# BigCiLeng/bilateral-driving

Measured on AMD Instinct MI355X. Metric: train iters/sec (fwd+bwd) at 2M Gaussians, 6x1920x1080; HBM roofline %, higher is better.
Workload: dtype f32

## Files before the change

bilateral_driving_amd/csrc/tiles.hip:

```cpp
#include "bds_common.h"
#include "gs_math.h"

namespace bds {

constexpr int kScanBlock = 256;
constexpr int kScanItems = 8;
constexpr int kScanTile = kScanBlock * kScanItems;

__device__ __forceinline__ uint32_t wave_incl_scan(uint32_t v) {
  const int lane = threadIdx.x & (kWave - 1);
#pragma unroll
  for (int o = 1; o < kWave; o <<= 1) {
    uint32_t t = __shfl_up(v, o);
    if (lane >= o) v += t;
  }
  return v;
}

__device__ __forceinline__ uint32_t block_excl_scan(uint32_t v, uint32_t &total, uint32_t *lds_w ) {
  const int lane = threadIdx.x & (kWave - 1), wv = threadIdx.x / kWave;
  const int nw = blockDim.x / kWave;
  uint32_t inc = wave_incl_scan(v);
  if (lane == kWave - 1) lds_w[wv] = inc;
  __syncthreads();
// ... 378 lines not shown
          gt[u] += c;
          if (g < gb) below[u] += c;
        }
      }
      const uint32_t *hp = hist + ((int64_t)gb << kWideGroupShift) * kBins + tid * kPer;
      const int nrows = vb - (gb << kWideGroupShift);
      uint32_t p0[kPer], p1[kPer], p2[kPer], p3[kPer];
#pragma unroll
      for (int u = 0; u < kPer; u++) { p0[u] = 0; p1[u] = 0; p2[u] = 0; p3[u] = 0; }
      int r = 0;
      for (; r + 4 <= nrows; r += 4) {
        const uint32_t *q = hp + (int64_t)r * kBins;
#pragma unroll
        for (int u = 0; u < kPer; u++) { p0[u] += q[u]; p1[u] += q[kBins + u]; p2[u] += q[2 * kBins + u]; p3[u] += q[3 * kBins + u]; }
      }
      for (; r < nrows; r++) {
#pragma unroll
        for (int u = 0; u < kPer; u++) p0[u] += hp[(int64_t)r * kBins + u];
      }
#pragma unroll
      for (int u = 0; u < kPer; u++) below[u] += (p0[u] + p1[u]) + (p2[u] + p3[u]);
    }
    uint32_t gsum = 0;
#pragma unroll
    for (int u = 0; u < kPer; u++) gsum += gt[u];
    uint32_t all;
    uint32_t dbase = block_excl_scan(gsum, all, lw);
    uint32_t base = block_excl_scan(sum, all, lw);
#pragma unroll
    for (int u = 0; u < kPer; u++) {
      const int d = tid * kPer + u;
      dstart[d] = base;
      gbase[d] = dbase + below[u];
      dbase += gt[u];
      if (offsets_out && vb == 0 && d < n_offsets) offsets_out[d] = (int32_t)gbase[d];
      uint32_t b2 = base;
#pragma unroll
      for (int w = 0; w < kSortWaves; w++) {
        const uint32_t c = wrun[w][d];
        wrun[w][d] = b2;
        b2 += c;
      }
      base += tot[u];
    }
  }
  __syncthreads();
  const unsigned long long lt = lane == 0 ? 0ull : (~0ull >> (64 - lane));
#pragma unroll
  for (int r = 0; r < kSortRounds; r++) {
    const int64_t i = wbase + r * kWave + lane;
    const bool on = i < n;
    const uint32_t d = (k[r] >> shift) & mask;
    unsigned long long peers = __ballot(on);
    for (int b = 0; b < bits; b++) {
      const unsigned long long bal = __ballot((d >> b) & 1u);
      peers &= ((d >> b) & 1u) ? bal : ~bal;
    }
    const uint32_t rank = __popcll(peers & lt);
    uint32_t pos = 0;
    if (on) pos = wrun[wv][d];
    __builtin_amdgcn_s_waitcnt(0xc07f);
    __builtin_amdgcn_wave_barrier();
    if (on && rank == 0) wrun[wv][d] = pos + __popcll(peers);
    __builtin_amdgcn_wave_barrier();
    if (on) lk[pos + rank] = k[r];
  }
  __syncthreads();
  const int cnt = (int)((n - bbase) < (int64_t)kSortChunk ? (n - bbase) : (int64_t)kSortChunk);
  for (int i = tid; i < cnt; i += kSortBlock) {
    const uint32_t kk = lk[i];
    const uint32_t d = (kk >> shift) & mask;
    const uint32_t g = gbase[d] + ((uint32_t)i - dstart[d]);
    keys_out[g] = kk;
    if (unpack) vals_out[g] = unpack[kk & rank_mask];
  }
}
template <int kBins>
__global__ __launch_bounds__(kSortBlock) void radix_scatter_keys_wide_kernel(
    const uint32_t *__restrict__ keys_in, int64_t n_host, const uint64_t *__restrict__ n_dev, int shift, uint32_t mask, int bits,
    const uint32_t *__restrict__ hist, const uint32_t *__restrict__ ghist, uint32_t *__restrict__ keys_out,
    const uint32_t *__restrict__ unpack, uint32_t rank_mask, uint32_t *__restrict__ vals_out, int32_t *__restrict__ offsets_out,
    int n_offsets) {
  __shared__ ScatterWideSh<kBins> sh;
  radix_scatter_keys_wide_block<kBins>(sh, (int)blockIdx.x, keys_in, list_length(n_host, n_dev), shift, mask, bits, hist, ghist, keys_out,
                                       unpack, rank_mask, vals_out, offsets_out, n_offsets);
}

constexpr int kWideBits = 10;

static size_t radix_temp_elems(int64_t n, int max_bins = 256) {
  const int64_t nblocks = cdiv(n > 0 ? n : 1, kSortChunk);
  const size_t h = align_up((size_t)max_bins * nblocks, 4);
  const size_t group_rows = max_bins > 256 ? (size_t)max_bins * (size_t)cdiv(nblocks, 1 << kWideGroupShift) : 0;
  const size_t behind = scan_temp_elems((int64_t)max_bins * nblocks);
  return h + (behind > group_rows ? behind : group_rows);
}

static size_t radix_wide_group_elems(int64_t n, int bits) {
  return (size_t)(1 << bits) * (size_t)cdiv(cdiv(n > 0 ? n : 1, kSortChunk), 1 << kWideGroupShift);
}

static int radix_pass(const uint32_t *kin, const uint32_t *vin, uint32_t *kout, uint32_t *vout, int64_t n, int shift,
                      int bits, uint32_t *temp, hipStream_t st, const uint64_t *n_dev = nullptr) {
  if (n == 0) return BDS_OK;
  const int nblocks = (int)cdiv(n, kSortChunk);
  const uint32_t mask = (1u << bits) - 1u;
  const int64_t hn = (int64_t)(mask + 1) * nblocks;
  uint32_t *hist = temp;
  uint32_t *stemp = temp + align_up((size_t)256 * nblocks, 4);
  hipLaunchKernelGGL(radix_hist_kernel, dim3(nblocks), dim3(kSortBlock), 0, st, kin, n, n_dev, shift, mask, nblocks, hist);
  BDS_LAUNCH_CHECK();
  int rc = exclusive_scan_u32(hist, hist, hn, stemp, nullptr, st);
  if (rc != BDS_OK) return rc;
  hipLaunchKernelGGL(radix_scatter_lds_kernel, dim3(nblocks), dim3(kSortBlock), 0, st, kin, vin, n, n_dev, shift, mask, bits,
                     nblocks, hist, kout, vout);
  BDS_LAUNCH_CHECK();
  return BDS_OK;
}


static int radix_pass_keys(const uint32_t *kin, uint32_t *kout, int64_t n, int shift, int bits, uint32_t *temp, hipStream_t st,
                           const uint32_t *unpack, uint32_t rank_mask, uint32_t *vout, int32_t *offsets_out = nullptr,
                           int n_offsets = 0, const uint64_t *n_dev = nullptr) {
  if (n == 0) return BDS_OK;
  const int nblocks = (int)cdiv(n, kSortChunk);
  const uint32_t mask = (1u << bits) - 1u;
  const int64_t hn = (int64_t)(mask + 1) * nblocks;
  uint32_t *hist = temp;
  uint32_t *stemp = temp + align_up((size_t)(bits > 8 ? (1 << kWideBits) : 256) * nblocks, 4);
  if (bits > 8) {
    uint32_t *ghist = stemp;
    if (bits == 9) {
      hipLaunchKernelGGL((radix_hist_wide_kernel<512>), dim3(nblocks), dim3(kSortBlock), 0, st, kin, n, n_dev, shift, mask, hist, ghist);
      hipLaunchKernelGGL((radix_scatter_keys_wide_kernel<512>), dim3(nblocks), dim3(kSortBlock), 0, st, kin, n, n_dev, shift, mask, bits,
                         hist, ghist, kout, unpack, rank_mask, vout, offsets_out, n_offsets);
    } else {
      hipLaunchKernelGGL((radix_hist_wide_kernel<1024>), dim3(nblocks), dim3(kSortBlock), 0, st, kin, n, n_dev, shift, mask, hist, ghist);
      hipLaunchKernelGGL((radix_scatter_keys_wide_kernel<1024>), dim3(nblocks), dim3(kSortBlock), 0, st, kin, n, n_dev, shift, mask, bits,
                         hist, ghist, kout, unpack, rank_mask, vout, offsets_out, n_offsets);
    }
    BDS_LAUNCH_CHECK();
    return BDS_OK;
  }
  hipLaunchKernelGGL(radix_hist_kernel, dim3(nblocks), dim3(kSortBlock), 0, st, kin, n, n_dev, shift, mask, nblocks, hist);
  BDS_LAUNCH_CHECK();
  int rc = exclusive_scan_u32(hist, hist, hn, stemp, nullptr, st);
  if (rc != BDS_OK) return rc;
  hipLaunchKernelGGL(radix_scatter_keys_kernel, dim3(nblocks), dim3(kSortBlock), 0, st, kin, n, n_dev, shift, mask, bits, nblocks,
                     hist, kout, unpack, rank_mask, vout);
  BDS_LAUNCH_CHECK();
  return BDS_OK;
}

constexpr int kGroupShift = 6;
constexpr int kShortRounds = 4;
constexpr int kShortChunk = kSortBlock * kShortRounds;
constexpr int kChunkShift = 10;
static_assert(kShortChunk == (1 << kChunkShift), "chunk shift");
constexpr int64_t kShortSortMax = (int64_t)kShortChunk * 8192;

struct ShortHistSh { uint32_t h[256]; };
__device__ __forceinline__ void short_hist_block(ShortHistSh &sh, int vb, const uint32_t *keys, int64_t n, int shift,
                                                 uint32_t *hist , uint32_t *ghist ) {
  const int64_t base = (int64_t)vb * kShortChunk;
  if (base >= n) return;
  sh.h[threadIdx.x] = 0;
  __syncthreads();
#pragma unroll 4
  for (int r = 0; r < kShortRounds; r++) {
    const int64_t i = base + r * kSortBlock + threadIdx.x;
    if (i < n) atomicAdd(&sh.h[(keys[i] >> shift) & 255u], 1u);
  }
  __syncthreads();
  const uint32_t c = sh.h[threadIdx.x];
  hist[(int64_t)vb * 256 + threadIdx.x] = c;
  if (c) atomicAdd(&ghist[(int64_t)(vb >> kGroupShift) * 256 + threadIdx.x], c);
}
__device__ __forceinline__ int64_t bounded_count(const uint64_t *n_dev, int64_t n_cap) {
  const int64_t n = (int64_t)*n_dev;
  return (n_cap >= 0 && n > n_cap) ? 0 : n;
}
__global__ __launch_bounds__(kSortBlock) void short_hist_kernel(const uint32_t *__restrict__ keys,
                                                               const uint64_t *__restrict__ n_dev, int64_t n_cap, int shift,
                                                               uint32_t *__restrict__ hist ,
                                                               uint32_t *__restrict__ ghist ) {
  __shared__ ShortHistSh sh;
  short_hist_block(sh, (int)blockIdx.x, keys, bounded_count(n_dev, n_cap), shift, hist, ghist);
}

struct ShortScatterSh {
  uint32_t wrun[kSortWaves][256];
  uint32_t lw[kSortBlock / kWave + 1];
};
__device__ __forceinline__ void short_scatter_block(ShortScatterSh &sh, int vb, const uint32_t *keys_in, const uint32_t *vals_in, int64_t n,
                                                    int shift, const uint32_t *hist, const uint32_t *ghist, uint32_t *keys_out,
                                                    uint32_t *vals_out) {
  if ((int64_t)vb * kShortChunk >= n) return;
  auto &wrun = sh.wrun;
  uint32_t *lw = sh.lw;
  const int tid = threadIdx.x, lane = tid & (kWave - 1), wv = tid / kWave;
#pragma unroll
  for (int w = 0; w < kSortWaves; w++) wrun[w][tid] = 0;
  const int nb = (int)((n + kShortChunk - 1) >> kChunkShift), ng = (nb + (1 << kGroupShift) - 1) >> kGroupShift;
  const int gb = vb >> kGroupShift;
  uint32_t below = 0, total = 0;
  {
    int g = 0;
    for (; g + 4 <= ng; g += 4) {
      const uint32_t *q = ghist + (int64_t)g * 256 + tid;
      const uint32_t c0 = q[0], c1 = q[256], c2 = q[512], c3 = q[768];
      total += (c0 + c1) + (c2 + c3);
      below += (g < gb ? c0 : 0u) + (g + 1 < gb ? c1 : 0u) + (g + 2 < gb ? c2 : 0u) + (g + 3 < gb ? c3 : 0u);
    }
    for (; g < ng; g++) {
      const uint32_t c = ghist[(int64_t)g * 256 + tid];
      total += c;
      if (g < gb) below += c;
    }
  }
  {
    const uint32_t *hp = hist + ((int64_t)gb << kGroupShift) * 256 + tid;
    const int nrows = vb - (gb << kGroupShift);
    uint32_t p0 = 0, p1 = 0, p2 = 0, p3 = 0, p4 = 0, p5 = 0, p6 = 0, p7 = 0;
    int r = 0;
    for (; r + 8 <= nrows; r += 8) {
      const uint32_t *q = hp + (int64_t)r * 256;
      const uint32_t a0 = q[0], a1 = q[256], a2 = q[512], a3 = q[768], a4 = q[1024], a5 = q[1280], a6 = q[1536], a7 = q[1792];
      p0 += a0; p1 += a1; p2 += a2; p3 += a3; p4 += a4; p5 += a5; p6 += a6; p7 += a7;
    }
    for (; r < nrows; r++) p0 += hp[(int64_t)r * 256];
    below += ((p0 + p1) + (p2 + p3)) + ((p4 + p5) + (p6 + p7));
  }
  uint32_t all;
  const uint32_t digit_base = block_excl_scan(total, all, lw);
  constexpr int kPerWave = kShortChunk / kSortWaves;
  const int64_t wbase = (int64_t)vb * kShortChunk + (int64_t)wv * kPerWave;
  uint32_t k[kShortRounds], v[kShortRounds];
#pragma unroll
  for (int r = 0; r < kShortRounds; r++) {
    const int64_t i = wbase + r * kWave + lane;
    k[r] = 0xFFFFFFFFu; v[r] = 0;
    if (i < n) {
      k[r] = keys_in[i]; v[r] = vals_in[i];
      atomicAdd(&wrun[wv][(k[r] >> shift) & 255u], 1u);
    }
  }
  __syncthreads();
  {
    uint32_t base = digit_base + below;
#pragma unroll
    for (int w = 0; w < kSortWaves; w++) {
      const uint32_t c = wrun[w][tid];
      wrun[w][tid] = base;
      base += c;
    }
  }
  __syncthreads();
  const unsigned long long lt = lane == 0 ? 0ull : (~0ull >> (64 - lane));
#pragma unroll
  for (int r = 0; r < kShortRounds; r++) {
    const int64_t i = wbase + r * kWave + lane;
    const bool on = i < n;
    const uint32_t d = (k[r] >> shift) & 255u;
    unsigned long long peers = __ballot(on);
#pragma unroll
    for (int b = 0; b < 8; b++) {
      const unsigned long long bal = __ballot((d >> b) & 1u);
      peers &= ((d >> b) & 1u) ? bal : ~bal;
    }
    const uint32_t rank = __popcll(peers & lt);
    uint32_t pos = 0;
    if (on) pos = wrun[wv][d];
    __builtin_amdgcn_s_waitcnt(0xc07f);
    __builtin_amdgcn_wave_barrier();
    if (on && rank == 0) wrun[wv][d] = pos + __popcll(peers);
    __builtin_amdgcn_wave_barrier();
    if (on) {
      keys_out[pos + rank] = k[r];
      vals_out[pos + rank] = v[r];
    }
  }
}
__global__ __launch_bounds__(kSortBlock) void short_scatter_kernel(
    const uint32_t *__restrict__ keys_in, const uint32_t *__restrict__ vals_in, const uint64_t *__restrict__ n_dev, int64_t n_cap,
    int shift, const uint32_t *__restrict__ hist, const uint32_t *__restrict__ ghist, uint32_t *__restrict__ keys_out,
    uint32_t *__restrict__ vals_out) {
  __shared__ ShortScatterSh sh;
  short_scatter_block(sh, (int)blockIdx.x, keys_in, vals_in, bounded_count(n_dev, n_cap), shift, hist, ghist, keys_out, vals_out);
}

static size_t short_sort_elems(int64_t n_bound) {
  const int64_t nb = cdiv(n_bound > 0 ? n_bound : 1, kShortChunk), ng = cdiv(nb, 1 << kGroupShift);
  return (size_t)(nb + 4 * ng) * 256;
}

constexpr int kIsectBlock = 256;

__global__ __launch_bounds__(kIsectBlock) void isect_flag_kernel(int64_t CN, const int32_t *__restrict__ radii,
                                                                uint32_t *__restrict__ flags) {
  const int64_t o = (int64_t)blockIdx.x * kIsectBlock + threadIdx.x;
  if (o < CN) flags[o] = radii[o] > 0 ? 1u : 0u;
}

__global__ __launch_bounds__(kIsectBlock) void isect_compact_kernel(int64_t CN, const int32_t *__restrict__ radii,
                                                                   const uint32_t *__restrict__ pos,
                                                                   const float *__restrict__ depths,
                                                                   uint32_t *__restrict__ keys, uint32_t *__restrict__ vals,
                                                                   uint32_t *__restrict__ asc, int compact, int sd) {
  const int64_t o = (int64_t)blockIdx.x * kIsectBlock + threadIdx.x;
  if (o >= CN || radii[o] <= 0) return;
  const uint32_t j = pos[o];
  keys[j] = __float_as_uint(depths[o * sd]);
  vals[j] = compact ? j : (uint32_t)o;
  asc[j] = (uint32_t)o;
}

__global__ __launch_bounds__(kScanBlock) void visible_reduce_kernel(int64_t CN, const int32_t *__restrict__ radii,
                                                                   uint32_t *__restrict__ tile_sums,
                                                                   uint32_t *__restrict__ zero_me, int64_t zero_elems,
                                                                   uint64_t *__restrict__ m_total, int32_t *__restrict__ zero_cn) {
  __shared__ uint32_t lw[kScanBlock / kWave + 1];
  if (blockIdx.x == 0 && threadIdx.x == 0) *m_total = 0;
  for (int64_t i = (int64_t)blockIdx.x * kScanBlock + threadIdx.x; i < zero_elems; i += (int64_t)gridDim.x * kScanBlock)
    zero_me[i] = 0u;
  const int64_t base = (int64_t)blockIdx.x * kScanTile + (int64_t)threadIdx.x * kScanItems;
  uint32_t s = 0;
#pragma unroll
  for (int i = 0; i < kScanItems; i++) {
    if (base + i < CN) {
      s += radii[base + i] > 0 ? 1u : 0u;
      if (zero_cn) zero_cn[base + i] = 0;
    }
  }
  uint32_t tot;
  block_excl_scan(s, tot, lw);
  if (threadIdx.x == 0) tile_sums[blockIdx.x] = tot;
}

constexpr int kCompactSpan = kScanTile / kShortChunk + 1;
struct VisCompactSh {
  uint32_t lw[kScanBlock / kWave + 1];
  uint32_t h[kCompactSpan][256];
};
__device__ __forceinline__ void visible_compact_block(VisCompactSh &sh, int vb, int nvb, int64_t CN, const int32_t *radii, const float *depths,
                                                      const uint32_t *tile_sums, uint32_t *keys, uint32_t *vals, uint32_t *hist,
                                                      uint32_t *ghist, uint64_t *n_vis_out, uint32_t *asc, int compact, int sums_per_tile,
                                                      int sd) {
  constexpr int kSpan = kCompactSpan;
  uint32_t *lw = sh.lw;
  auto &h = sh.h;
#pragma unroll
  for (int t = 0; t < kSpan; t++) h[t][threadIdx.x] = 0;
  uint32_t part = 0;
  for (int b = threadIdx.x; b < vb * sums_per_tile; b += kScanBlock) part += tile_sums[b];
  uint32_t my_offset;
  block_excl_scan(part, my_offset, lw);
  const int64_t base = (int64_t)vb * kScanTile + (int64_t)threadIdx.x * kScanItems;
  bool vis[kScanItems];
  uint32_t s = 0;
#pragma unroll
  for (int i = 0; i < kScanItems; i++) {
    vis[i] = base + i < CN && radii[base + i] > 0;
    s += vis[i] ? 1u : 0u;
  }
  uint32_t tot;
  uint32_t j = block_excl_scan(s, tot, lw) + my_offset;
  const uint32_t chunk0 = my_offset >> kChunkShift;
#pragma unroll
  for (int i = 0; i < kScanItems; i++) {
    if (vis[i]) {
      const uint32_t key = __float_as_uint(depths[(base + i) * sd]);
      keys[j] = key;
      vals[j] = compact ? j : (uint32_t)(base + i);
      asc[j] = (uint32_t)(base + i);
      atomicAdd(&h[(j >> kChunkShift) - chunk0][key & 255u], 1u);
      j++;
    }
  }
  __syncthreads();
#pragma unroll
  for (int t = 0; t < kSpan; t++) {
    const uint32_t c = h[t][threadIdx.x];
    if (c) {
      atomicAdd(&hist[(int64_t)(chunk0 + t) * 256 + threadIdx.x], c);
      atomicAdd(&ghist[(int64_t)((chunk0 + t) >> kGroupShift) * 256 + threadIdx.x], c);
    }
  }
  if (vb == nvb - 1 && threadIdx.x == 0) *n_vis_out = (uint64_t)my_offset + tot;
}
__global__ __launch_bounds__(kScanBlock) void visible_compact_kernel(int64_t CN, const int32_t *__restrict__ radii,
                                                                    const float *__restrict__ depths,
                                                                    const uint32_t *__restrict__ tile_sums,
                                                                    uint32_t *__restrict__ keys, uint32_t *__restrict__ vals,
                                                                    uint32_t *__restrict__ hist, uint32_t *__restrict__ ghist,
                                                                    uint64_t *__restrict__ n_vis_out, uint32_t *__restrict__ asc,
                                                                    int compact, int sums_per_tile, int sd) {
  __shared__ VisCompactSh sh;
  visible_compact_block(sh, (int)blockIdx.x, (int)gridDim.x, CN, radii, depths, tile_sums, keys, vals, hist, ghist, n_vis_out, asc, compact,
                        sums_per_tile, sd);
}

struct RowStage {
  float mx[kIsectBlock], my[kIsectBlock], a[kIsectBlock], b[kIsectBlock], c[kIsectBlock], qmax[kIsectBlock];
  int x0[kIsectBlock], x1[kIsectBlock], y0[kIsectBlock];
  uint32_t id[kIsectBlock];
  uint32_t cam_base[kIsectBlock];
  uint32_t rowoff[kIsectBlock + 1];
  uint32_t lw[kIsectBlock / kWave + 1];
};

constexpr int kRecWords = 12;

__device__ __forceinline__ uint32_t stage_rows(RowStage &S, int64_t j0, int64_t n_vis, int64_t N, const uint32_t *__restrict__ sorted_idx,
                                               const uint32_t *__restrict__ asc ,
                                               const float *__restrict__ means2d, const int32_t *__restrict__ radii,
                                               const float *__restrict__ conics, const float *__restrict__ opacities,
                                               int tile_size, int tile_w, int tile_h, float4 *__restrict__ rec_out,
                                               const float4 *__restrict__ rec_in, const ProjLayout pl) {
  const int t = threadIdx.x;
  const int64_t j = j0 + t;
  uint32_t nrows = 0;
  if (j < n_vis) {
    if (rec_in != nullptr) {
      const float4 r0 = rec_in[j * 3], r1 = rec_in[j * 3 + 1], r2 = rec_in[j * 3 + 2];
      nrows = __float_as_uint(r2.y);
      S.mx[t] = r0.x; S.my[t] = r0.y; S.a[t] = r0.z; S.b[t] = r0.w;
      S.c[t] = r1.x; S.qmax[t] = r1.y; S.x0[t] = __float_as_int(r1.z); S.x1[t] = __float_as_int(r1.w);
      S.y0[t] = __float_as_int(r2.x); S.id[t] = __float_as_uint(r2.z); S.cam_base[t] = __float_as_uint(r2.w);
    } else {
      const uint32_t val = sorted_idx[j];
      const uint32_t o = asc ? asc[val] : val;
      const int r = proj_radius(pl, means2d, radii, (int64_t)o);
      float mx = means2d[(int64_t)o * pl.s2], my = means2d[(int64_t)o * pl.s2 + 1];
      float a = 0.f, b = 0.f, c = 0.f, q_max = 0.f, op = 0.f;
      if (conics != nullptr) {
        a = conics[(int64_t)o * pl.sc]; b = conics[(int64_t)o * pl.sc + 1]; c = conics[(int64_t)o * pl.sc + 2];
        op = opacities[(int64_t)o * pl.so];
      }
      int x0 = 0, y0 = 0, x1 = 0, y1 = 0;
      if (r > 0) {
        bool ok;
        if (conics == nullptr) {
          tile_rect(mx, my, r, tile_size, tile_w, tile_h, x0, y0, x1, y1);
          ok = x1 > x0 && y1 > y0;
        } else {
          ok = tile_rect_tight(mx, my, r, a, b, c, op, tile_size, tile_w, tile_h, x0, y0, x1, y1, q_max);
        }
        if (ok) nrows = (uint32_t)(y1 - y0);
      } else {
        mx = my = a = b = c = 0.f;
      }
      const uint32_t cam_base = (int64_t)o < N ? 0u : (uint32_t)((uint32_t)o / (uint32_t)N) * (uint32_t)(tile_w * tile_h);
      S.mx[t] = mx; S.my[t] = my; S.a[t] = a; S.b[t] = b; S.c[t] = c; S.qmax[t] = q_max;
      S.x0[t] = x0; S.x1[t] = x1; S.y0[t] = y0; S.id[t] = val; S.cam_base[t] = cam_base;
      if (rec_out != nullptr) {
        rec_out[j * 3] = make_float4(mx, my, a, b);
        rec_out[j * 3 + 1] = make_float4(c, q_max, __int_as_float(x0), __int_as_float(x1));
        rec_out[j * 3 + 2] = make_float4(__int_as_float(y0), __uint_as_float(nrows), __uint_as_float(val), __uint_as_float(cam_base));
      }
    }
  }
  uint32_t total;
  const uint32_t ex = block_excl_scan(nrows, total, S.lw);
  S.rowoff[t] = ex;
  if (t == 0) S.rowoff[kIsectBlock] = total;
  __syncthreads();
  return total;
}

__device__ __forceinline__ int row_owner(const RowStage &S, uint32_t r) {
  int lo = 0, hi = kIsectBlock;
#pragma unroll
  for (int s = 0; s < 8; s++) {
    const int mid = (lo + hi) >> 1;
    if (S.rowoff[mid] <= r) lo = mid; else hi = mid;
  }
  return lo;
}

__device__ __forceinline__ void row_span_of(const RowStage &S, int g, int ty, bool cull, int tile_size, int &lo, int &hi) {
  lo = S.x0[g]; hi = S.x1[g];
  if (cull) row_tile_span(S.mx[g], S.my[g], S.a[g], S.b[g], S.c[g], S.qmax[g], ty, tile_size, S.x0[g], S.x1[g], lo, hi);
}

struct CountRowsSh {
  RowStage S;
  uint32_t cnt[kIsectBlock];
};
__device__ __forceinline__ void isect_count_rows_block(CountRowsSh &sh, int vb, int64_t n_vis, const uint32_t *sorted_idx, const float *means2d,
                                                       const int32_t *radii, const float *conics, const float *opacities, int tile_size,
                                                       int tile_w, int tile_h, int32_t *tiles_per_gauss, int64_t N, float4 *rec,
                                                       uint32_t *btot, const uint32_t *asc, const ProjLayout pl) {
  RowStage &S = sh.S;
  uint32_t *cnt = sh.cnt;
  const int64_t j0 = (int64_t)vb * kIsectBlock, j = j0 + threadIdx.x;
  if (j0 >= n_vis) {
    if (threadIdx.x == 0) btot[vb] = 0u;
    return;
  }
  cnt[threadIdx.x] = 0u;
  const uint32_t R = stage_rows(S, j0, n_vis, N, sorted_idx, asc, means2d, radii, conics, opacities, tile_size, tile_w, tile_h, rec, nullptr, pl);
  const bool cull = conics != nullptr;
  for (uint32_t r = threadIdx.x; r < R; r += kIsectBlock) {
    const int g = row_owner(S, r);
    int lo, hi;
    row_span_of(S, g, S.y0[g] + (int)(r - S.rowoff[g]), cull, tile_size, lo, hi);
    if (hi > lo) atomicAdd(&cnt[g], (uint32_t)(hi - lo));
  }
  __syncthreads();
  if (tiles_per_gauss && j < n_vis) tiles_per_gauss[asc ? asc[sorted_idx[j]] : sorted_idx[j]] = (int32_t)cnt[threadIdx.x];
  uint32_t total;
  block_excl_scan(cnt[threadIdx.x], total, S.lw);
  if (threadIdx.x == 0) btot[vb] = total;
}
__global__ __launch_bounds__(kIsectBlock) void isect_count_rows_kernel(
    const uint64_t *__restrict__ n_vis_dev, int64_t n_cap, const uint32_t *__restrict__ sorted_idx, const float *__restrict__ means2d,
    const int32_t *__restrict__ radii, const float *__restrict__ conics, const float *__restrict__ opacities, int tile_size,
    int tile_w, int tile_h, int32_t *__restrict__ tiles_per_gauss, int64_t N, float4 *__restrict__ rec, uint32_t *__restrict__ btot,
    const uint32_t *__restrict__ asc, const ProjLayout pl) {
  __shared__ CountRowsSh sh;
  isect_count_rows_block(sh, (int)blockIdx.x, bounded_count(n_vis_dev, n_cap), sorted_idx, means2d, radii, conics, opacities, tile_size, tile_w, tile_h,
                         tiles_per_gauss, N, rec, btot, asc, pl);
}

struct EmitRowsSh { RowStage S; };
__device__ __forceinline__ void isect_emit_rows_block(EmitRowsSh &sh, int vb, int64_t n_vis, int64_t N, const uint32_t *sorted_idx,
                                                      const uint32_t *btot, const float *means2d, const int32_t *radii, const float *conics,
                                                      const float *opacities, int tile_size, int tile_w, int tile_h, uint32_t *keys,
                                                      uint32_t *vals, int pack_shift, const float4 *rec) {
  RowStage &S = sh.S;
  const int64_t j0 = (int64_t)vb * kIsectBlock;
  if (j0 >= n_vis) return;
  const uint32_t R = stage_rows(S, j0, n_vis, N, sorted_idx, nullptr, means2d, radii, conics, opacities, tile_size, tile_w, tile_h, nullptr, rec,
                                ProjLayout{2, 1, 3, 1, 0});
  const bool cull = conics != nullptr;
  uint32_t carry;
  {
    uint32_t part = 0;
// ... 62 lines not shown

struct PrepWs {
  uint64_t *total;
  uint32_t *ka, *va, *kb, *vb;
  uint32_t *cum;
  uint32_t *asc;
  uint32_t *temp;
  uint32_t *tables;
  float4 *rec;
  uint32_t *btot;
  size_t bytes;
};

static PrepWs prep_layout(void *ws, int64_t CN) {
  PrepWs L;
  char *p = static_cast<char *>(ws);
  size_t off = 0;
  auto take = [&](size_t elems, size_t esz) {
    char *q = p ? p + off : nullptr;
    off += align_up(elems * esz, 256);
    return q;
  };
  L.total = reinterpret_cast<uint64_t *>(take(8, 8));
  L.ka = reinterpret_cast<uint32_t *>(take(CN, 4));
  L.va = reinterpret_cast<uint32_t *>(take(CN, 4));
  L.kb = reinterpret_cast<uint32_t *>(take(CN, 4));
  L.vb = reinterpret_cast<uint32_t *>(take(CN, 4));
  L.cum = reinterpret_cast<uint32_t *>(take(CN, 4));
  L.asc = reinterpret_cast<uint32_t *>(take(CN, 4));
  size_t t = radix_temp_elems(CN);
  size_t t2 = scan_temp_elems(CN);
  L.temp = reinterpret_cast<uint32_t *>(take(t > t2 ? t : t2, 4));
  L.tables = reinterpret_cast<uint32_t *>(take(CN <= kShortSortMax ? short_sort_elems(CN) : 0, 4));
  L.rec = reinterpret_cast<float4 *>(take((size_t)CN * kRecWords, 4));
  L.btot = reinterpret_cast<uint32_t *>(take((size_t)cdiv(CN > 0 ? CN : 1, kIsectBlock) + 1, 4));
  L.bytes = off;
  return L;
}

struct BuildWs {
  uint32_t *ka, *va, *kb;
  uint32_t *temp;
  size_t bytes;
};

static BuildWs build_layout(void *ws, int64_t M) {
  BuildWs L;
  char *p = static_cast<char *>(ws);
  size_t off = 0;
  auto take = [&](size_t elems, size_t esz) {
    char *q = p ? p + off : nullptr;
    off += align_up(elems * esz, 256);
    return q;
  };
  L.ka = reinterpret_cast<uint32_t *>(take(M, 4));
  L.va = reinterpret_cast<uint32_t *>(take(M, 4));
  L.kb = reinterpret_cast<uint32_t *>(take(M, 4));
  L.temp = reinterpret_cast<uint32_t *>(take(radix_temp_elems(M, 1 << kWideBits), 4));
  L.bytes = off + 256;
  return L;
}

}

using namespace bds;

int bds::prep_reduce_slots(void *ws, size_t ws_bytes, int64_t CN, PrepReduceSlots *out) {
  BDS_REQUIRE(ws && out && CN > 0 && CN < (int64_t)1 << 31);
  if (!(CN <= kShortSortMax && option_get(kOptShortSort))) return BDS_ECAPACITY;
  PrepWs L = prep_layout(ws, CN);
  if (ws_bytes < L.bytes) return BDS_EWORKSPACE;
  out->sums256 = L.temp;
  out->zero_me = L.tables;
  out->zero_elems = (int64_t)short_sort_elems(CN);
  out->m_total = L.total;
  return BDS_OK;
}

extern "C" size_t bds_isect_visible_ids_offset(int C, int64_t N) {
  if (C < 1 || N < 0) return 0;
  char *const base = reinterpret_cast<char *>(static_cast<uintptr_t>(4096));
  const PrepWs L = prep_layout(base, (int64_t)C * N);
  return static_cast<size_t>(reinterpret_cast<char *>(L.asc) - base);
}

extern "C" size_t bds_isect_prepare_workspace_bytes(int C, int64_t N) {
  if (C < 1 || N < 0) return 0;
  return prep_layout(nullptr, (int64_t)C * N).bytes;
}

extern "C" size_t bds_isect_build_workspace_bytes(int C, int64_t N, int64_t M) {
  (void)C; (void)N;
  if (M < 0) return 0;
  return build_layout(nullptr, M).bytes;
}

constexpr int kCountMEff = 2, kCountVisEff = 3, kCountOverflow = 4;
__global__ __launch_bounds__(256) void finish_counts_kernel(const uint32_t *__restrict__ btot, int nblocks, uint64_t *__restrict__ counts_dev,
                                                           volatile int64_t *__restrict__ counts_host, int64_t cap_m, int64_t cap_vis) {
  __shared__ unsigned long long part[256];
  unsigned long long s0 = 0, s1 = 0, s2 = 0, s3 = 0;
  int b = threadIdx.x;
  for (; b + 768 < nblocks; b += 1024) {
    const uint32_t a0 = btot[b], a1 = btot[b + 256], a2 = btot[b + 512], a3 = btot[b + 768];
    s0 += a0; s1 += a1; s2 += a2; s3 += a3;
  }
  for (; b < nblocks; b += 256) s0 += btot[b];
  part[threadIdx.x] = (s0 + s1) + (s2 + s3);
  __syncthreads();
  for (int o = 128; o > 0; o >>= 1) {
    if ((int)threadIdx.x < o) part[threadIdx.x] += part[threadIdx.x + o];
    __syncthreads();
  }
  if (threadIdx.x == 0) {
    counts_dev[0] = part[0];
    const uint64_t nv = counts_dev[1];
    if (cap_m >= 0) {
      const bool over = (int64_t)part[0] > cap_m || (int64_t)nv > cap_vis;
      counts_dev[kCountMEff] = over ? 0ull : part[0];
      counts_dev[kCountVisEff] = over ? 0ull : nv;
      counts_dev[kCountOverflow] = over ? 1ull : 0ull;
      if (counts_host && over) counts_host[2] = 1;
    }
    if (counts_host) { counts_host[0] = (int64_t)part[0]; counts_host[1] = (int64_t)nv; }
  }
  if (counts_host) __threadfence_system();
}

static int prepare_enqueue(int C, int64_t N, const float *means2d, const int32_t *radii, const float *depths,
                           const float *conics, const float *opacities, int tile_size, int tile_w, int tile_h,
                           int32_t *tiles_per_gauss, void *ws, size_t ws_bytes, int compact, bds_stream_t stream,
                           uint64_t **counts_dev, const uint32_t **btot_out, int *nblocks_out, int64_t nvis_bound = -1) {
  BDS_REQUIRE(C >= 1 && N >= 0 && tile_size > 0 && tile_w > 0 && tile_h > 0);
  const int64_t CN = (int64_t)C * N;
  BDS_REQUIRE(CN < (int64_t)1 << 31);
  BDS_REQUIRE((int64_t)C * tile_w * tile_h < (int64_t)1 << 31);
  *counts_dev = nullptr;
  *btot_out = nullptr; *nblocks_out = 0;
  if (CN == 0) return BDS_OK;
  BDS_REQUIRE(means2d && radii && depths && ws);
  BDS_REQUIRE((conics == nullptr) == (opacities == nullptr));
  const ProjLayout pl = proj_layout(means2d, depths, conics, opacities);
  PrepWs L = prep_layout(ws, CN);
  if (ws_bytes < L.bytes) return BDS_EWORKSPACE;
  hipStream_t st = as_stream(stream);
  if (nvis_bound < 0 || nvis_bound > CN || !option_get(kOptCapLaunch)) nvis_bound = CN;
  const int64_t n_cap = nvis_bound < CN ? nvis_bound : (int64_t)-1;
  const unsigned grid = (unsigned)cdiv(nvis_bound > 0 ? nvis_bound : 1, kIsectBlock);
  uint64_t *n_vis = L.total + 1;
  int rc;
  if (CN <= kShortSortMax && option_get(kOptShortSort)) {
    const int64_t nb = cdiv(CN, kShortChunk), ng = cdiv(nb, 1 << kGroupShift);
    const unsigned nb_launch = (unsigned)cdiv(nvis_bound > 0 ? nvis_bound : 1, kShortChunk);
    uint32_t *hist = L.tables, *ghist = L.tables + nb * 256;
    const unsigned tiles = (unsigned)cdiv(CN, kScanTile);
    if (!(compact & 2))
      hipLaunchKernelGGL(visible_reduce_kernel, dim3(tiles), dim3(kScanBlock), 0, st, CN, radii, L.temp, L.tables,
                         (int64_t)short_sort_elems(CN), L.total, tiles_per_gauss);
    hipLaunchKernelGGL(visible_compact_kernel, dim3(tiles), dim3(kScanBlock), 0, st, CN, radii, depths, L.temp, L.ka, L.va, hist,
                       ghist, n_vis, L.asc, compact & 1, (compact & 2) ? kScanTile / 256 : 1, pl.sd);
    BDS_LAUNCH_CHECK();
    uint32_t *kin = L.ka, *vin = L.va, *kout = L.kb, *vout = L.vb;
    for (int p = 0; p < 4; p++) {
      uint32_t *gh = ghist + (int64_t)p * ng * 256;
      if (p > 0) hipLaunchKernelGGL(short_hist_kernel, dim3(nb_launch), dim3(kSortBlock), 0, st, kin, n_vis, n_cap, 8 * p, hist, gh);
      hipLaunchKernelGGL(short_scatter_kernel, dim3(nb_launch), dim3(kSortBlock), 0, st, kin, vin, n_vis, n_cap, 8 * p, hist, gh, kout,
                         vout);
      uint32_t *t;
      t = kin; kin = kout; kout = t;
      t = vin; vin = vout; vout = t;
    }
    BDS_LAUNCH_CHECK();
    hipLaunchKernelGGL(isect_count_rows_kernel, dim3(grid), dim3(kIsectBlock), 0, st, n_vis, n_cap, L.va, means2d, radii, conics,
                       opacities, tile_size, tile_w, tile_h, tiles_per_gauss, N, L.rec, L.btot,
                       (compact & 1) ? L.asc : (const uint32_t *)nullptr, pl);
    BDS_LAUNCH_CHECK();
  } else {
    BDS_REQUIRE(!(compact & 2));
    if (hipMemsetAsync(L.total, 0, sizeof(uint64_t), st) != hipSuccess) return BDS_ELAUNCH;
    hipLaunchKernelGGL(isect_flag_kernel, dim3(grid), dim3(kIsectBlock), 0, st, CN, radii, L.kb);
    BDS_LAUNCH_CHECK();
    rc = exclusive_scan_u32(L.kb, L.cum, CN, L.temp, n_vis, st);
    if (rc != BDS_OK) return rc;
    hipLaunchKernelGGL(isect_compact_kernel, dim3(grid), dim3(kIsectBlock), 0, st, CN, radii, L.cum, depths, L.ka, L.va, L.asc, compact, pl.sd);
    BDS_LAUNCH_CHECK();
    uint32_t *kin = L.ka, *vin = L.va, *kout = L.kb, *vout = L.vb;
    for (int p = 0; p < 4; p++) {
      rc = radix_pass(kin, vin, kout, vout, CN, 8 * p, 8, L.temp, st, n_vis);
      if (rc != BDS_OK) return rc;
      uint32_t *t;
      t = kin; kin = kout; kout = t;
      t = vin; vin = vout; vout = t;
    }
    if (tiles_per_gauss && hipMemsetAsync(tiles_per_gauss, 0, sizeof(int32_t) * CN, st) != hipSuccess) return BDS_ELAUNCH;
    hipLaunchKernelGGL(isect_count_rows_kernel, dim3(grid), dim3(kIsectBlock), 0, st, n_vis, (int64_t)-1, L.va, means2d, radii, conics,
                       opacities, tile_size, tile_w, tile_h, tiles_per_gauss, N, L.rec, L.btot,
                       compact ? L.asc : (const uint32_t *)nullptr, pl);
    BDS_LAUNCH_CHECK();
  }
  (void)rc;
  *counts_dev = L.total;
  *btot_out = L.btot; *nblocks_out = (int)grid;
  return BDS_OK;
}

extern "C" int bds_isect_prepare(int C, int64_t N, const float *means2d, const int32_t *radii, const float *depths,
                                 const float *conics, const float *opacities, int tile_size, int tile_w, int tile_h,
                                 int32_t *tiles_per_gauss, void *ws, size_t ws_bytes, int64_t M_capacity, int64_t n_visible_capacity,
                                 int64_t *counts, void *event, int compact, bds_stream_t stream) {
  BDS_REQUIRE((M_capacity < 0) == (n_visible_capacity < 0));
  const bool dev = M_capacity >= 0, sync = !dev && !event;
  if (dev) {
    BDS_REQUIRE(!event && (int64_t)C * N > 0);
  } else {
    BDS_REQUIRE(counts);
    counts[0] = 0; counts[1] = 0;
  }
  uint64_t *counts_dev = nullptr;
  const uint32_t *btot = nullptr;
  int nblocks = 0;
  int rc = prepare_enqueue(C, N, means2d, radii, depths, conics, opacities, tile_size, tile_w, tile_h, tiles_per_gauss, ws, ws_bytes,
                           compact, stream, &counts_dev, &btot, &nblocks, dev ? n_visible_capacity : (int64_t)-1);
  if (rc != BDS_OK) return rc;
  hipStream_t st = as_stream(stream);
  if (counts_dev != nullptr) {
    void *mapped = nullptr;
    if (!sync && counts && hipHostGetDevicePointer(&mapped, counts, 0) != hipSuccess) {
      (void)hipGetLastError();
      if (dev) return BDS_EINVAL;
      mapped = nullptr;
    }
    hipLaunchKernelGGL(finish_counts_kernel, dim3(1), dim3(256), 0, st, btot, nblocks, counts_dev, static_cast<volatile int64_t *>(mapped),
                       M_capacity, n_visible_capacity);
    BDS_LAUNCH_CHECK();
    if (!dev && mapped == nullptr &&
        hipMemcpyAsync(counts, counts_dev, 2 * sizeof(uint64_t), hipMemcpyDeviceToHost, st) != hipSuccess)
      return BDS_ELAUNCH;
    if (sync && hipStreamSynchronize(st) != hipSuccess) return BDS_ELAUNCH;
  }
  if (event && hipEventRecord(static_cast<hipEvent_t>(event), st) != hipSuccess) return BDS_ELAUNCH;
  return BDS_OK;
}

extern "C" size_t bds_isect_counts_offset(int which) {
  return (which >= 0 && which <= kCountOverflow) ? (size_t)which * sizeof(uint64_t) : (size_t)0;
}

extern "C" int bds_isect_build(int C, int64_t N, int64_t M, int64_t n_visible, const float *means2d, const int32_t *radii,
                               const float *depths, const float *conics, const float *opacities, int tile_size,
                               int tile_w, int tile_h, const void *ws,
                               size_t ws_bytes, void *ws2, size_t ws2_bytes, int64_t *isect_ids, int32_t *flatten_ids,
                               int32_t *isect_offsets, int32_t *visible_ids, int device_counts, int compact, bds_stream_t stream) {
  const bool dev = device_counts != 0;
  if (dev) BDS_REQUIRE(M > 0 && n_visible > 0 && !isect_ids && !visible_ids);
  BDS_REQUIRE(C >= 1 && N >= 0 && M >= 0 && tile_size > 0 && tile_w > 0 && tile_h > 0 && isect_offsets);
  BDS_REQUIRE(!(compact && isect_ids));
  BDS_REQUIRE(!visible_ids || n_visible >= 0);
  if (visible_ids && n_visible > 0) {
    BDS_REQUIRE(ws);
    const PrepWs P0 = prep_layout(const_cast<void *>(ws), (int64_t)C * N);
    if (ws_bytes < P0.bytes) return BDS_EWORKSPACE;
    if (hipMemcpyAsync(visible_ids, P0.asc, sizeof(int32_t) * n_visible, hipMemcpyDeviceToDevice, as_stream(stream)) != hipSuccess)
      return BDS_ELAUNCH;
  }
  BDS_REQUIRE(M < (int64_t)1 << 31);
  const int64_t CN = (int64_t)C * N;
  const int n_tiles_total = C * tile_w * tile_h;
  hipStream_t st = as_stream(stream);
  if (M == 0) {
    if (hipMemsetAsync(isect_offsets, 0, sizeof(int32_t) * n_tiles_total, st) != hipSuccess) return BDS_ELAUNCH;
    return BDS_OK;
  }
  BDS_REQUIRE(means2d && radii && depths && ws && ws2 && flatten_ids);
  const ProjLayout pl = proj_layout(means2d, depths, conics, opacities);
  PrepWs P = prep_layout(const_cast<void *>(ws), CN);
  if (ws_bytes < P.bytes) return BDS_EWORKSPACE;
  const uint64_t *const M_dev = dev ? P.total + kCountMEff : nullptr;
  const uint64_t *const nvis_dev = dev ? P.total + kCountVisEff : P.total + 1;
  BuildWs B = build_layout(ws2, M);
  if (ws2_bytes < B.bytes) return BDS_EWORKSPACE;
  int nbits = 1;
  while (((int64_t)1 << nbits) < n_tiles_total) nbits++;
  BDS_REQUIRE((conics == nullptr) == (opacities == nullptr));
  uint32_t *fl = reinterpret_cast<uint32_t *>(flatten_ids);
  const int rank_bits = 32 - nbits;
  const bool packed = n_visible >= 0 && rank_bits >= 1 && n_visible <= ((int64_t)1 << rank_bits) && option_get(kOptPacked);
  if (dev && !packed) return BDS_ECAPACITY;
  const int max_digit = (packed && nbits > 8 && nbits <= kWideBits) ? kWideBits : 8;
  const int npass = (nbits + max_digit - 1) / max_digit;
  const int bits_per = (nbits + npass - 1) / npass;
  int key_shift = 0;
  bool offsets_fused = false;
  uint32_t *kin;
  if (packed) {
    key_shift = rank_bits;
    uint32_t *k_emit = (npass % 2 == 1) ? B.ka : B.kb;
    const bool wide = bits_per > 8;
    uint32_t *wide_zero = wide ? B.temp + align_up((size_t)(1 << kWideBits) * (size_t)cdiv(M, kSortChunk), 4) : nullptr;
    const int wide_zero_n = wide ? (int)radix_wide_group_elems(M, bits_per) : 0;
    const int64_t emit_bound = (n_visible > 0 && n_visible < CN && option_get(kOptCapLaunch)) ? n_visible : CN;
    hipLaunchKernelGGL(isect_emit_rows_kernel, dim3((unsigned)cdiv(emit_bound, kIsectBlock)), dim3(kIsectBlock), 0, st, nvis_dev, N, P.va,
                       P.btot, means2d, radii, conics, opacities, tile_size, tile_w, tile_h, k_emit, (uint32_t *)nullptr, rank_bits, P.rec,
                       wide_zero, wide_zero_n);
    BDS_LAUNCH_CHECK();
    kin = k_emit;
    const uint32_t rank_mask = (1u << rank_bits) - 1u;
    for (int p = 0; p < npass; p++) {
      uint32_t *kout = (kin == B.ka) ? B.kb : B.ka;
      int bits = bits_per;
      if (bits_per * (p + 1) > nbits) bits = nbits - bits_per * p;
      const bool last = p == npass - 1;
      offsets_fused = npass == 1 && bits > 8 && !isect_ids;
      int rc = radix_pass_keys(kin, kout, M, rank_bits + bits_per * p, bits, B.temp, st, last ? P.va : nullptr, rank_mask,
                               last ? fl : nullptr, offsets_fused ? isect_offsets : nullptr, n_tiles_total, M_dev);
      if (rc != BDS_OK) return rc;
      kin = kout;
    }
  } else {
    uint32_t *k_emit, *v_emit;
    if (npass % 2 == 1) { k_emit = B.ka; v_emit = B.va; }
    else { k_emit = B.kb; v_emit = fl; }
    hipLaunchKernelGGL(isect_emit_rows_kernel, dim3((unsigned)cdiv(CN, kIsectBlock)), dim3(kIsectBlock), 0, st, P.total + 1, N,
                       P.va, P.btot, means2d, radii, conics, opacities, tile_size, tile_w, tile_h, k_emit, v_emit, 0, P.rec,
                       (uint32_t *)nullptr, 0);
    BDS_LAUNCH_CHECK();
// ... 42 lines not shown
```

Baseline: 1090.

## Switch visible-Gaussian depth sort to three 11-bit radix passes with larger chunks

Replaces the four 8-bit LSD radix passes in the short sort with three passes of 11/11/10 bits. Chunks grow to 4096 elements per block and groups shrink to 16 blocks. Histograms become 2048-bin, and prefix reads use uint4 loads with each thread owning 8 digits. Wave-local digit counts are now built from ballot peer masks rather than one LDS atomic per element. The aim is to cut one full read/write pass over keys and values plus one launch pair, at the cost of more LDS, larger histogram tables, extra ballots per element and a lower maximum size for the short path.

```diff
diff --git a/bilateral_driving_amd/csrc/tiles.hip b/bilateral_driving_amd/csrc/tiles.hip
--- a/bilateral_driving_amd/csrc/tiles.hip
+++ b/bilateral_driving_amd/csrc/tiles.hip
@@ -554,87 +554,73 @@
   return BDS_OK;
 }
 
-constexpr int kGroupShift = 6;
-constexpr int kShortRounds = 4;
+constexpr int kGroupShift = 4;
+constexpr int kShortRounds = 16;
 constexpr int kShortChunk = kSortBlock * kShortRounds;
-constexpr int kChunkShift = 10;
+constexpr int kChunkShift = 12;
 static_assert(kShortChunk == (1 << kChunkShift), "chunk shift");
-constexpr int64_t kShortSortMax = (int64_t)kShortChunk * 8192;
-
-struct ShortHistSh { uint32_t h[256]; };
-__device__ __forceinline__ void short_hist_block(ShortHistSh &sh, int vb, const uint32_t *keys, int64_t n, int shift,
+constexpr int64_t kShortSortMax = (int64_t)kShortChunk * 2048;
+constexpr int kShortPasses = 3;
+constexpr int kShortDigitBits = 11;
+constexpr int kShortBins = 1 << kShortDigitBits;
+constexpr int kShortPer = kShortBins / kSortBlock;
+static_assert(kShortPer == 8, "two uint4 per thread and row");
+static inline int short_digit_bits(int p) { return p + 1 < kShortPasses ? kShortDigitBits : 32 - kShortDigitBits * (kShortPasses - 1); }
+
+struct ShortHistSh { uint32_t h[kShortBins]; };
+__device__ __forceinline__ void short_hist_block(ShortHistSh &sh, int vb, const uint32_t *keys, int64_t n, int shift, int bits,
                                                  uint32_t *hist , uint32_t *ghist ) {
   const int64_t base = (int64_t)vb * kShortChunk;
   if (base >= n) return;
-  sh.h[threadIdx.x] = 0;
+  const uint32_t mask = (1u << bits) - 1u;
+  for (int d = threadIdx.x; d < kShortBins; d += kSortBlock) sh.h[d] = 0;
   __syncthreads();
 #pragma unroll 4
   for (int r = 0; r < kShortRounds; r++) {
     const int64_t i = base + r * kSortBlock + threadIdx.x;
-    if (i < n) atomicAdd(&sh.h[(keys[i] >> shift) & 255u], 1u);
-  }
-  __syncthreads();
-  const uint32_t c = sh.h[threadIdx.x];
-  hist[(int64_t)vb * 256 + threadIdx.x] = c;
-  if (c) atomicAdd(&ghist[(int64_t)(vb >> kGroupShift) * 256 + threadIdx.x], c);
+    if (i < n) atomicAdd(&sh.h[(keys[i] >> shift) & mask], 1u);
+  }
+  __syncthreads();
+  for (int d = threadIdx.x; d <= (int)mask; d += kSortBlock) {
+    const uint32_t c = sh.h[d];
+    hist[(int64_t)vb * kShortBins + d] = c;
+    if (c) atomicAdd(&ghist[(int64_t)(vb >> kGroupShift) * kShortBins + d], c);
+  }
 }
 __device__ __forceinline__ int64_t bounded_count(const uint64_t *n_dev, int64_t n_cap) {
   const int64_t n = (int64_t)*n_dev;
   return (n_cap >= 0 && n > n_cap) ? 0 : n;
 }
 __global__ __launch_bounds__(kSortBlock) void short_hist_kernel(const uint32_t *__restrict__ keys,
-                                                               const uint64_t *__restrict__ n_dev, int64_t n_cap, int shift,
+                                                               const uint64_t *__restrict__ n_dev, int64_t n_cap, int shift, int bits,
                                                                uint32_t *__restrict__ hist ,
                                                                uint32_t *__restrict__ ghist ) {
   __shared__ ShortHistSh sh;
-  short_hist_block(sh, (int)blockIdx.x, keys, bounded_count(n_dev, n_cap), shift, hist, ghist);
+  short_hist_block(sh, (int)blockIdx.x, keys, bounded_count(n_dev, n_cap), shift, bits, hist, ghist);
 }
 
 struct ShortScatterSh {
-  uint32_t wrun[kSortWaves][256];
+  alignas(16) uint32_t wrun[kSortWaves][kShortBins];
   uint32_t lw[kSortBlock / kWave + 1];
 };
+__device__ __forceinline__ void add_row(uint32_t (&acc)[kShortPer], const uint4 a, const uint4 b) {
+  acc[0] += a.x; acc[1] += a.y; acc[2] += a.z; acc[3] += a.w;
+  acc[4] += b.x; acc[5] += b.y; acc[6] += b.z; acc[7] += b.w;
+}
 __device__ __forceinline__ void short_scatter_block(ShortScatterSh &sh, int vb, const uint32_t *keys_in, const uint32_t *vals_in, int64_t n,
-                                                    int shift, const uint32_t *hist, const uint32_t *ghist, uint32_t *keys_out,
+                                                    int shift, int bits, const uint32_t *hist, const uint32_t *ghist, uint32_t *keys_out,
                                                     uint32_t *vals_out) {
   if ((int64_t)vb * kShortChunk >= n) return;
   auto &wrun = sh.wrun;
   uint32_t *lw = sh.lw;
   const int tid = threadIdx.x, lane = tid & (kWave - 1), wv = tid / kWave;
-#pragma unroll
-  for (int w = 0; w < kSortWaves; w++) wrun[w][tid] = 0;
-  const int nb = (int)((n + kShortChunk - 1) >> kChunkShift), ng = (nb + (1 << kGroupShift) - 1) >> kGroupShift;
-  const int gb = vb >> kGroupShift;
-  uint32_t below = 0, total = 0;
-  {
-    int g = 0;
-    for (; g + 4 <= ng; g += 4) {
-      const uint32_t *q = ghist + (int64_t)g * 256 + tid;
-      const uint32_t c0 = q[0], c1 = q[256], c2 = q[512], c3 = q[768];
-      total += (c0 + c1) + (c2 + c3);
-      below += (g < gb ? c0 : 0u) + (g + 1 < gb ? c1 : 0u) + (g + 2 < gb ? c2 : 0u) + (g + 3 < gb ? c3 : 0u);
-    }
-    for (; g < ng; g++) {
-      const uint32_t c = ghist[(int64_t)g * 256 + tid];
-      total += c;
-      if (g < gb) below += c;
-    }
-  }
-  {
-    const uint32_t *hp = hist + ((int64_t)gb << kGroupShift) * 256 + tid;
-    const int nrows = vb - (gb << kGroupShift);
-    uint32_t p0 = 0, p1 = 0, p2 = 0, p3 = 0, p4 = 0, p5 = 0, p6 = 0, p7 = 0;
-    int r = 0;
-    for (; r + 8 <= nrows; r += 8) {
-      const uint32_t *q = hp + (int64_t)r * 256;
-      const uint32_t a0 = q[0], a1 = q[256], a2 = q[512], a3 = q[768], a4 = q[1024], a5 = q[1280], a6 = q[1536], a7 = q[1792];
-      p0 += a0; p1 += a1; p2 += a2; p3 += a3; p4 += a4; p5 += a5; p6 += a6; p7 += a7;
-    }
-    for (; r < nrows; r++) p0 += hp[(int64_t)r * 256];
-    below += ((p0 + p1) + (p2 + p3)) + ((p4 + p5) + (p6 + p7));
-  }
-  uint32_t all;
-  const uint32_t digit_base = block_excl_scan(total, all, lw);
+  const uint32_t mask = (1u << bits) - 1u;
+#pragma unroll
+  for (int w = 0; w < kSortWaves; w++) {
+    uint4 *z = reinterpret_cast<uint4 *>(&wrun[w][tid * kShortPer]);
+    z[0] = make_uint4(0, 0, 0, 0);
+    z[1] = make_uint4(0, 0, 0, 0);
+  }
   constexpr int kPerWave = kShortChunk / kSortWaves;
   const int64_t wbase = (int64_t)vb * kShortChunk + (int64_t)wv * kPerWave;
   uint32_t k[kShortRounds], v[kShortRounds];
@@ -642,40 +628,90 @@
   for (int r = 0; r < kShortRounds; r++) {
     const int64_t i = wbase + r * kWave + lane;
     k[r] = 0xFFFFFFFFu; v[r] = 0;
-    if (i < n) {
-      k[r] = keys_in[i]; v[r] = vals_in[i];
-      atomicAdd(&wrun[wv][(k[r] >> shift) & 255u], 1u);
-    }
-  }
-  __syncthreads();
-  {
-    uint32_t base = digit_base + below;
-#pragma unroll
-    for (int w = 0; w < kSortWaves; w++) {
-      const uint32_t c = wrun[w][tid];
-      wrun[w][tid] = base;
-      base += c;
-    }
-  }
-  __syncthreads();
+    if (i < n) { k[r] = keys_in[i]; v[r] = vals_in[i]; }
+  }
+  uint32_t below[kShortPer], total[kShortPer];
+#pragma unroll
+  for (int u = 0; u < kShortPer; u++) { below[u] = 0; total[u] = 0; }
+  if (tid * kShortPer <= (int)mask) {
+    const int nb = (int)((n + kShortChunk - 1) >> kChunkShift), ng = (nb + (1 << kGroupShift) - 1) >> kGroupShift;
+    const int gb = vb >> kGroupShift;
+    const uint4 *gq = reinterpret_cast<const uint4 *>(ghist + tid * kShortPer);
+    constexpr int kRow4 = kShortBins / 4;
+    int g = 0;
+    for (; g + 2 <= ng; g += 2) {
+      const uint4 a0 = gq[(int64_t)g * kRow4], b0 = gq[(int64_t)g * kRow4 + 1];
+      const uint4 a1 = gq[(int64_t)(g + 1) * kRow4], b1 = gq[(int64_t)(g + 1) * kRow4 + 1];
+      add_row(total, a0, b0); add_row(total, a1, b1);
+      if (g < gb) add_row(below, a0, b0);
+      if (g + 1 < gb) add_row(below, a1, b1);
+    }
+    for (; g < ng; g++) {
+      const uint4 a0 = gq[(int64_t)g * kRow4], b0 = gq[(int64_t)g * kRow4 + 1];
+      add_row(total, a0, b0);
+      if (g < gb) add_row(below, a0, b0);
+    }
+    const uint4 *hq = reinterpret_cast<const uint4 *>(hist + ((int64_t)gb << kGroupShift) * kShortBins + tid * kShortPer);
+    const int nrows = vb - (gb << kGroupShift);
+    int r = 0;
+    for (; r + 4 <= nrows; r += 4) {
+      const uint4 a0 = hq[(int64_t)r * kRow4], b0 = hq[(int64_t)r * kRow4 + 1];
+      const uint4 a1 = hq[(int64_t)(r + 1) * kRow4], b1 = hq[(int64_t)(r + 1) * kRow4 + 1];
+      const uint4 a2 = hq[(int64_t)(r + 2) * kRow4], b2 = hq[(int64_t)(r + 2) * kRow4 + 1];
+      const uint4 a3 = hq[(int64_t)(r + 3) * kRow4], b3 = hq[(int64_t)(r + 3) * kRow4 + 1];
+      add_row(below, a0, b0); add_row(below, a1, b1); add_row(below, a2, b2); add_row(below, a3, b3);
+    }
+    for (; r < nrows; r++) add_row(below, hq[(int64_t)r * kRow4], hq[(int64_t)r * kRow4 + 1]);
+  }
+  uint32_t mine = 0;
+#pragma unroll
+  for (int u = 0; u < kShortPer; u++) mine += total[u];
+  uint32_t all;
+  uint32_t digit_base = block_excl_scan(mine, all, lw);
   const unsigned long long lt = lane == 0 ? 0ull : (~0ull >> (64 - lane));
+  uint32_t rk[kShortRounds];
 #pragma unroll
   for (int r = 0; r < kShortRounds; r++) {
-    const int64_t i = wbase + r * kWave + lane;
-    const bool on = i < n;
-    const uint32_t d = (k[r] >> shift) & 255u;
+    const bool on = wbase + r * kWave + lane < n;
+    const uint32_t d = (k[r] >> shift) & mask;
     unsigned long long peers = __ballot(on);
 #pragma unroll
-    for (int b = 0; b < 8; b++) {
+    for (int b = 0; b < kShortDigitBits - 1; b++) {
       const unsigned long long bal = __ballot((d >> b) & 1u);
       peers &= ((d >> b) & 1u) ? bal : ~bal;
     }
-    const uint32_t rank = __popcll(peers & lt);
+    if (bits == kShortDigitBits) {
+      const unsigned long long bal = __ballot((d >> (kShortDigitBits - 1)) & 1u);
+      peers &= ((d >> (kShortDigitBits - 1)) & 1u) ? bal : ~bal;
+    }
+    const uint32_t rank = __popcll(peers & lt), cnt = __popcll(peers);
+    rk[r] = rank | (cnt << 8);
+    if (on && rank == 0) atomicAdd(&wrun[wv][d], cnt);
+  }
+  __syncthreads();
+#pragma unroll
+  for (int u = 0; u < kShortPer; u++) {
+    const int d = tid * kShortPer + u;
+    uint32_t base = digit_base + below[u];
+#pragma unroll
+    for (int w = 0; w < kSortWaves; w++) {
+      const uint32_t c = wrun[w][d];
+      wrun[w][d] = base;
+      base += c;
+    }
+    digit_base += total[u];
+  }
+  __syncthreads();
+#pragma unroll
+  for (int r = 0; r < kShortRounds; r++) {
+    const bool on = wbase + r * kWave + lane < n;
+    const uint32_t d = (k[r] >> shift) & mask;
+    const uint32_t rank = rk[r] & 255u;
     uint32_t pos = 0;
     if (on) pos = wrun[wv][d];
     __builtin_amdgcn_s_waitcnt(0xc07f);
     __builtin_amdgcn_wave_barrier();
-    if (on && rank == 0) wrun[wv][d] = pos + __popcll(peers);
+    if (on && rank == 0) wrun[wv][d] = pos + (rk[r] >> 8);
     __builtin_amdgcn_wave_barrier();
     if (on) {
       keys_out[pos + rank] = k[r];
@@ -685,15 +721,15 @@
 }
 __global__ __launch_bounds__(kSortBlock) void short_scatter_kernel(
     const uint32_t *__restrict__ keys_in, const uint32_t *__restrict__ vals_in, const uint64_t *__restrict__ n_dev, int64_t n_cap,
-    int shift, const uint32_t *__restrict__ hist, const uint32_t *__restrict__ ghist, uint32_t *__restrict__ keys_out,
+    int shift, int bits, const uint32_t *__restrict__ hist, const uint32_t *__restrict__ ghist, uint32_t *__restrict__ keys_out,
     uint32_t *__restrict__ vals_out) {
   __shared__ ShortScatterSh sh;
-  short_scatter_block(sh, (int)blockIdx.x, keys_in, vals_in, bounded_count(n_dev, n_cap), shift, hist, ghist, keys_out, vals_out);
+  short_scatter_block(sh, (int)blockIdx.x, keys_in, vals_in, bounded_count(n_dev, n_cap), shift, bits, hist, ghist, keys_out, vals_out);
 }
 
 static size_t short_sort_elems(int64_t n_bound) {
   const int64_t nb = cdiv(n_bound > 0 ? n_bound : 1, kShortChunk), ng = cdiv(nb, 1 << kGroupShift);
-  return (size_t)(nb + 4 * ng) * 256;
+  return (size_t)(nb + kShortPasses * ng) * kShortBins;
 }
 
 constexpr int kIsectBlock = 256;
@@ -739,10 +775,10 @@
   if (threadIdx.x == 0) tile_sums[blockIdx.x] = tot;
 }
 
-constexpr int kCompactSpan = kScanTile / kShortChunk + 1;
+constexpr int kCompactSpan = (kScanTile + kShortChunk - 2) / kShortChunk + 1;
 struct VisCompactSh {
   uint32_t lw[kScanBlock / kWave + 1];
-  uint32_t h[kCompactSpan][256];
+  uint32_t h[kCompactSpan][kShortBins];
 };
 __device__ __forceinline__ void visible_compact_block(VisCompactSh &sh, int vb, int nvb, int64_t CN, const int32_t *radii, const float *depths,
                                                       const uint32_t *tile_sums, uint32_t *keys, uint32_t *vals, uint32_t *hist,
@@ -752,7 +788,8 @@
   uint32_t *lw = sh.lw;
   auto &h = sh.h;
 #pragma unroll
-  for (int t = 0; t < kSpan; t++) h[t][threadIdx.x] = 0;
+  for (int t = 0; t < kSpan; t++)
+    for (int d = threadIdx.x; d < kShortBins; d += kScanBlock) h[t][d] = 0;
   uint32_t part = 0;
   for (int b = threadIdx.x; b < vb * sums_per_tile; b += kScanBlock) part += tile_sums[b];
   uint32_t my_offset;
@@ -775,17 +812,19 @@
       keys[j] = key;
       vals[j] = compact ? j : (uint32_t)(base + i);
       asc[j] = (uint32_t)(base + i);
-      atomicAdd(&h[(j >> kChunkShift) - chunk0][key & 255u], 1u);
+      atomicAdd(&h[(j >> kChunkShift) - chunk0][key & (uint32_t)(kShortBins - 1)], 1u);
       j++;
     }
   }
   __syncthreads();
 #pragma unroll
   for (int t = 0; t < kSpan; t++) {
-    const uint32_t c = h[t][threadIdx.x];
-    if (c) {
-      atomicAdd(&hist[(int64_t)(chunk0 + t) * 256 + threadIdx.x], c);
-      atomicAdd(&ghist[(int64_t)((chunk0 + t) >> kGroupShift) * 256 + threadIdx.x], c);
+    for (int d = threadIdx.x; d < kShortBins; d += kScanBlock) {
+      const uint32_t c = h[t][d];
+      if (c) {
+        atomicAdd(&hist[(int64_t)(chunk0 + t) * kShortBins + d], c);
+        atomicAdd(&ghist[(int64_t)((chunk0 + t) >> kGroupShift) * kShortBins + d], c);
+      }
     }
   }
   if (vb == nvb - 1 && threadIdx.x == 0) *n_vis_out = (uint64_t)my_offset + tot;
@@ -1154,25 +1193,28 @@
   if (CN <= kShortSortMax && option_get(kOptShortSort)) {
     const int64_t nb = cdiv(CN, kShortChunk), ng = cdiv(nb, 1 << kGroupShift);
     const unsigned nb_launch = (unsigned)cdiv(nvis_bound > 0 ? nvis_bound : 1, kShortChunk);
-    uint32_t *hist = L.tables, *ghist = L.tables + nb * 256;
+    uint32_t *hist = L.tables, *ghist = L.tables + nb * kShortBins;
+    uint32_t *kin = (kShortPasses & 1) ? L.kb : L.ka, *vin = (kShortPasses & 1) ? L.vb : L.va;
+    uint32_t *kout = (kShortPasses & 1) ? L.ka : L.kb, *vout = (kShortPasses & 1) ? L.va : L.vb;
     const unsigned tiles = (unsigned)cdiv(CN, kScanTile);
     if (!(compact & 2))
       hipLaunchKernelGGL(visible_reduce_kernel, dim3(tiles), dim3(kScanBlock), 0, st, CN, radii, L.temp, L.tables,
                          (int64_t)short_sort_elems(CN), L.total, tiles_per_gauss);
-    hipLaunchKernelGGL(visible_compact_kernel, dim3(tiles), dim3(kScanBlock), 0, st, CN, radii, depths, L.temp, L.ka, L.va, hist,
+    hipLaunchKernelGGL(visible_compact_kernel, dim3(tiles), dim3(kScanBlock), 0, st, CN, radii, depths, L.temp, kin, vin, hist,
                        ghist, n_vis, L.asc, compact & 1, (compact & 2) ? kScanTile / 256 : 1, pl.sd);
     BDS_LAUNCH_CHECK();
-    uint32_t *kin = L.ka, *vin = L.va, *kout = L.kb, *vout = L.vb;
-    for (int p = 0; p < 4; p++) {
-      uint32_t *gh = ghist + (int64_t)p * ng * 256;
-      if (p > 0) hipLaunchKernelGGL(short_hist_kernel, dim3(nb_launch), dim3(kSortBlock), 0, st, kin, n_vis, n_cap, 8 * p, hist, gh);
-      hipLaunchKernelGGL(short_scatter_kernel, dim3(nb_launch), dim3(kSortBlock), 0, st, kin, vin, n_vis, n_cap, 8 * p, hist, gh, kout,
-                         vout);
+    for (int p = 0; p < kShortPasses; p++) {
+      uint32_t *gh = ghist + (int64_t)p * ng * kShortBins;
+      const int shift = kShortDigitBits * p, bits = short_digit_bits(p);
+      if (p > 0) hipLaunchKernelGGL(short_hist_kernel, dim3(nb_launch), dim3(kSortBlock), 0, st, kin, n_vis, n_cap, shift, bits, hist, gh);
+      hipLaunchKernelGGL(short_scatter_kernel, dim3(nb_launch), dim3(kSortBlock), 0, st, kin, vin, n_vis, n_cap, shift, bits, hist, gh,
+                         kout, vout);
       uint32_t *t;
       t = kin; kin = kout; kout = t;
       t = vin; vin = vout; vout = t;
     }
     BDS_LAUNCH_CHECK();
+    BDS_REQUIRE(kin == L.ka && vin == L.va);
     hipLaunchKernelGGL(isect_count_rows_kernel, dim3(grid), dim3(kIsectBlock), 0, st, n_vis, n_cap, L.va, means2d, radii, conics,
                        opacities, tile_size, tile_w, tile_h, tiles_per_gauss, N, L.rec, L.btot,
                        (compact & 1) ? L.asc : (const uint32_t *)nullptr, pl);
```

Result: slower. 1005 (-7.8%).
